# megapose6d/megapose6d

Measured on AMD Instinct MI355X. Metric: pose-hypotheses/sec (render+coarse+refine), 640×480, megapose-1.0-RGB, higher is better.
Workload: dtype f32 (results of fp32 arithmetic; the convolutions' multiplications run on the bf16 MFMA as EXACT piece products of the fp32 operands, fp32 accumulate)

## Files before the change

### megapose6d_amd/csrc/bf16x9_split.h

```cpp
#pragma once
#include <hip/hip_runtime.h>

#include <cstring>

namespace mp {

static inline void bf16x9_split3(float v, unsigned short out[3]) {
  unsigned vb, rb, qb;
  memcpy(&vb, &v, 4);
  const unsigned h = vb & 0xFFFF0000u;
  float hf; memcpy(&hf, &h, 4);
  const float r = v - hf;
  memcpy(&rb, &r, 4);
  const unsigned m = rb & 0xFFFF0000u;
  float mf; memcpy(&mf, &m, 4);
  const float q = r - mf;
  memcpy(&qb, &q, 4);
  out[0] = (unsigned short)(h >> 16); out[1] = (unsigned short)(m >> 16); out[2] = (unsigned short)(qb >> 16);
}

typedef unsigned bf16x9_u32x4 __attribute__((ext_vector_type(4)));

__device__ __forceinline__ void bf16x9_split8(const float4& lo, const float4& hi, bf16x9_u32x4 (&pc)[3]) {
  const float v[8] = {lo.x, lo.y, lo.z, lo.w, hi.x, hi.y, hi.z, hi.w};
  unsigned vb[8], rb[8], qb[8];
#pragma unroll
  for (int e = 0; e < 8; ++e) {
    vb[e] = __float_as_uint(v[e]);
    const float r = v[e] - __uint_as_float(vb[e] & 0xFFFF0000u);
    rb[e] = __float_as_uint(r);
    qb[e] = __float_as_uint(r - __uint_as_float(rb[e] & 0xFFFF0000u));
  }
#pragma unroll
  for (int j = 0; j < 4; ++j) {
    pc[0][j] = __builtin_amdgcn_perm(vb[2 * j + 1], vb[2 * j], 0x07060302u);
    pc[1][j] = __builtin_amdgcn_perm(rb[2 * j + 1], rb[2 * j], 0x07060302u);
    pc[2][j] = __builtin_amdgcn_perm(qb[2 * j + 1], qb[2 * j], 0x07060302u);
  }
}

}
```

### megapose6d_amd/csrc/conv_bf16x9.hip

```cpp
#include <cstdlib>

#include "bf16x9_split.h"
#include "conv_common.h"

namespace mp {

typedef __bf16 bf16x8 __attribute__((ext_vector_type(8)));
typedef bf16x9_u32x4 db_u32x4;

constexpr int DB_BM = 128, DB_BN = 128;
constexpr int DB_SLICE_BYTES = (DB_BN / 32) * 3 * 1024;
__device__ constexpr int DB_PA[9] = {2, 1, 2, 0, 1, 2, 0, 1, 0}, DB_PB[9] = {2, 2, 1, 2, 1, 0, 1, 0, 0};

__global__ __launch_bounds__(256) __attribute__((amdgpu_waves_per_eu(2, 2))) void conv_nhwc_bf16x9(ConvParams p) {
  __shared__ __attribute__((aligned(16))) float As[2 * DB_BM * LDS_LD];
  __shared__ int row_off[DB_BM];
  const int tid = threadIdx.x, lane = tid & 63;
  const int wave = __builtin_amdgcn_readfirstlane(tid >> 6);
  const int wm = wave >> 1, wn = wave & 1;
  const int lb = xcd_remap(blockIdx.x, gridDim.x);
  const int nblk = lb % p.n_nblocks, mblk = lb / p.n_nblocks;
  const int m0 = mblk * DB_BM, n0 = nblk * DB_BN;

  if (tid < DB_BM) {
    const int m = m0 + tid;
    int off = -1;
    if (m < p.M) {
      const int wo = m % p.Wo, t = m / p.Wo, ho = t % p.Ho, n = t / p.Ho;
      off = (((n * p.Hop) + ho + p.out_border) * p.Wop + wo + p.out_border) * p.Cout;
    }
    row_off[tid] = off;
  }
  const int a_c4 = tid & 7, a_r0 = tid >> 3;
  size_t pix[5];
#pragma unroll
  for (int i = 0; i < 5; ++i) {
    int m = i < 4 ? m0 + a_r0 + 32 * i : m0;
    m = m < p.M ? m : p.M - 1;
    const int wo = m % p.Wo, t = m / p.Wo, ho = t % p.Ho, n = t / p.Ho;
    pix[i] = ((size_t)n * p.Hp + (size_t)(ho * p.stride + p.in_off)) * p.Wp + (size_t)(wo * p.stride + p.in_off);
  }
  const __amdgpu_buffer_rsrc_t a_rsrc = __builtin_amdgcn_make_buffer_rsrc((void*)(p.x + pix[4] * p.C), 0, -1, 0x00020000);
  int a_voff[4];
#pragma unroll
  for (int i = 0; i < 4; ++i) a_voff[i] = (int)(((pix[i] - pix[4]) * p.C + a_c4 * 4) * 4);
  const __amdgpu_buffer_rsrc_t b_rsrc = __builtin_amdgcn_make_buffer_rsrc(
      (void*)(reinterpret_cast<const char*>(p.w) + (size_t)nblk * (2 * p.n_chunks) * DB_SLICE_BYTES), 0, -1, 0x00020000);
  const int b_voff = (2 * wn) * 3 * 1024 + lane * 16;

  f32x16 acc[2][2];
#pragma unroll
  for (int i = 0; i < 2; ++i)
#pragma unroll
    for (int j = 0; j < 2; ++j)
#pragma unroll
      for (int r = 0; r < 16; ++r) acc[i][j][r] = 0.f;

  float4 a0, a1, a2, a3;
  db_u32x4 bA[2][3], bB[2][3];
#define DB_BUF4(V, S) ([&] { const db_u32x4 v_ = __builtin_amdgcn_raw_buffer_load_b128(a_rsrc, V, S, 0);                  \
    return make_float4(__uint_as_float(v_.x), __uint_as_float(v_.y), __uint_as_float(v_.z), __uint_as_float(v_.w)); }())
#define DB_LOAD_A(SU)                       \
  a0 = DB_BUF4(a_voff[0], (SU) * 4);        \
  a1 = DB_BUF4(a_voff[1], (SU) * 4);        \
  a2 = DB_BUF4(a_voff[2], (SU) * 4);        \
  a3 = DB_BUF4(a_voff[3], (SU) * 4);
#define DB_LOAD_B(DST, SLICE)                                                                                       \
  _Pragma("unroll") for (int jl = 0; jl < 2; ++jl)                                                                  \
    _Pragma("unroll") for (int pc = 0; pc < 3; ++pc)                                                                \
      DST[jl][pc] = __builtin_amdgcn_raw_buffer_load_b128(b_rsrc, b_voff, (SLICE) * DB_SLICE_BYTES + (jl * 3 + pc) * 1024, 0);
#define DB_STORE_A(BUF)                                                            \
  {                                                                                \
    float* as_w = As + (BUF) * DB_BM * LDS_LD + a_r0 * LDS_LD + a_c4 * 4;          \
    *reinterpret_cast<float4*>(as_w) = a0;                                         \
    *reinterpret_cast<float4*>(as_w + 32 * LDS_LD) = a1;                           \
    *reinterpret_cast<float4*>(as_w + 64 * LDS_LD) = a2;                           \
    *reinterpret_cast<float4*>(as_w + 96 * LDS_LD) = a3;                           \
  }
#define DB_MFMA_SLICE(PA_, BB_)                                                                                     \
  _Pragma("unroll") for (int pr = 0; pr < 9; ++pr)                                                                  \
    _Pragma("unroll") for (int i = 0; i < 2; ++i)                                                                   \
      _Pragma("unroll") for (int j = 0; j < 2; ++j)                                                                 \
        acc[i][j] = __builtin_amdgcn_mfma_f32_32x32x16_bf16(__builtin_bit_cast(bf16x8, PA_[i][DB_PA[pr]]),          \
                                                            __builtin_bit_cast(bf16x8, BB_[j][DB_PB[pr]]), acc[i][j], 0, 0, 0);

  int a_su = 0, ju = 0;
  const int row_wrap = p.Wp * p.C - p.run;
  const int n_ch = p.n_chunks, last_slice = 2 * p.n_chunks - 1;
  DB_LOAD_A(0)
  DB_LOAD_B(bA, 0)
  DB_STORE_A(0)
  __syncthreads();

  const float* fr = As + (wm * 64 + (lane & 31)) * LDS_LD + (lane >> 5) * 8;
  for (int c = 0; c < n_ch; ++c) {
    const int buf = c & 1;
    if (c + 1 < n_ch) {
      a_su += BK;
      ju += BK;
      if (ju == p.run) { ju = 0; a_su += row_wrap; }
    }
    DB_LOAD_A(a_su)
    DB_LOAD_B(bB, 2 * c + 1)
    __builtin_amdgcn_sched_barrier(0);
    const float* fb = fr + buf * DB_BM * LDS_LD;
    float4 raw[2][2][2];
#pragma unroll
    for (int i = 0; i < 2; ++i) {
      raw[0][i][0] = *reinterpret_cast<const float4*>(fb + i * 32 * LDS_LD);
      raw[0][i][1] = *reinterpret_cast<const float4*>(fb + i * 32 * LDS_LD + 4);
    }
    db_u32x4 pa0[2][3], pa1[2][3];
    bf16x9_split8(raw[0][0][0], raw[0][0][1], pa0[0]);
    bf16x9_split8(raw[0][1][0], raw[0][1][1], pa0[1]);
    __builtin_amdgcn_sched_barrier(0);
#pragma unroll
    for (int i = 0; i < 2; ++i) {
      raw[1][i][0] = *reinterpret_cast<const float4*>(fb + i * 32 * LDS_LD + 16);
      raw[1][i][1] = *reinterpret_cast<const float4*>(fb + i * 32 * LDS_LD + 16 + 4);
    }
    DB_MFMA_SLICE(pa0, bA)
    bf16x9_split8(raw[1][0][0], raw[1][0][1], pa1[0]);
    bf16x9_split8(raw[1][1][0], raw[1][1][1], pa1[1]);
    __builtin_amdgcn_sched_group_barrier(0x100, 4, 0);
    __builtin_amdgcn_sched_group_barrier(0x008, 2, 0);
#pragma unroll
    for (int g = 0; g < 22; ++g) {
      __builtin_amdgcn_sched_group_barrier(0x002, 4, 0);
      __builtin_amdgcn_sched_group_barrier(0x008, 1, 0);
    }
    __builtin_amdgcn_sched_group_barrier(0x008, 12, 0);
    __builtin_amdgcn_sched_barrier(0);
    DB_LOAD_B(bA, (2 * c + 2 <= last_slice ? 2 * c + 2 : last_slice))
    DB_MFMA_SLICE(pa1, bB)
    DB_STORE_A(buf ^ 1)
    __syncthreads();
  }
#undef DB_BUF4
#undef DB_LOAD_A
#undef DB_LOAD_B
#undef DB_STORE_A
#undef DB_MFMA_SLICE

  const int erow0 = wm * 64 + (lane >> 5) * 4, en0 = n0 + wn * 64 + (lane & 31);
  const int emode = (p.residual ? 1 : 0) | (p.relu ? 2 : 0) | (p.y_act ? 4 : 0);
  switch (emode) {
    case 0: conv_epilogue<2, 2, false, false, false>(p, acc, row_off, erow0, en0); break;
    case 1: conv_epilogue<2, 2, true, false, false>(p, acc, row_off, erow0, en0); break;
    case 2: conv_epilogue<2, 2, false, true, false>(p, acc, row_off, erow0, en0); break;
    case 3: conv_epilogue<2, 2, true, true, false>(p, acc, row_off, erow0, en0); break;
    case 4: conv_epilogue<2, 2, false, false, true>(p, acc, row_off, erow0, en0); break;
    case 5: conv_epilogue<2, 2, true, false, true>(p, acc, row_off, erow0, en0); break;
    case 6: conv_epilogue<2, 2, false, true, true>(p, acc, row_off, erow0, en0); break;
    default: conv_epilogue<2, 2, true, true, true>(p, acc, row_off, erow0, en0); break;
  }
}

static int packed_slices(int Cin_p, int KH, int KW) { return 2 * ceil_div((long)KH * KW * Cin_p, BK); }

}

using namespace mp;

extern "C" size_t mp_conv_bf16x9_packed_bytes(int Cin_p, int Cout, int KH, int KW) {
  return (size_t)ceil_div(Cout, DB_BN) * packed_slices(Cin_p, KH, KW) * DB_SLICE_BYTES;
}

extern "C" int mp_conv_bf16x9_pack_weights(const float* w, int Cout, int Cin, int KH, int KW, int Cin_p, const float* scale, void* packed) {
  MP_REQUIRE(w && packed && Cout >= 1 && Cin >= 1 && KH >= 1 && KW >= 1 && Cin_p >= Cin && Cin_p % 16 == 0,
             "mp_conv_bf16x9_pack_weights: bad arguments (Cin_p %% 16 == 0, Cin_p >= Cin)");
  const int run = KW * Cin_p, k_total = KH * run, n_sl = packed_slices(Cin_p, KH, KW);
  unsigned short* out = (unsigned short*)packed;
  memset(out, 0, mp_conv_bf16x9_packed_bytes(Cin_p, Cout, KH, KW));
  for (int n = 0; n < Cout; ++n) {
    const float s = scale ? scale[n] : 1.f;
    const int nb = n / DB_BN, j = (n % DB_BN) / 32, nl = n % 32;
    for (int k = 0; k < k_total; ++k) {
      const int kh = k / run, jj = k % run, kw = jj / Cin_p, c = jj % Cin_p;
      if (c >= Cin) continue;
      unsigned short pc[3];
      bf16x9_split3(w[(((size_t)n * Cin + c) * KH + kh) * KW + kw] * s, pc);
      const int t = k / 16, lane = ((k % 16) / 8) * 32 + nl, e = k % 8;
      for (int piece = 0; piece < 3; ++piece)
        out[(((((size_t)nb * n_sl + t) * 4 + j) * 3 + piece) * 64 + lane) * 8 + e] = pc[piece];
    }
  }
  return MP_OK;
}

extern "C" int mp_conv2d_bf16x9_nhwc(const mp_conv_desc* desc, const void* d_w_pieces, mp_stream stream) {
  MP_REQUIRE(desc && d_w_pieces, "mp_conv2d_bf16x9_nhwc: null pointer");
  MP_REQUIRE(!desc->x_f16, "mp_conv2d_bf16x9_nhwc: fp32 input only");
  mp_conv_desc d = *desc;
  d.d_w = (const float*)d_w_pieces;
  ConvParams p;
  const int rc = conv_make_params(&d, &p);
  if (rc) return rc;
  MP_REQUIRE(d.C % 16 == 0 && p.run % BK == 0, "mp_conv2d_bf16x9_nhwc: needs C %% 16 == 0 and KW * C %% 32 == 0 (C = %d, KW = %d)", d.C, d.KW);
  p.n_mblocks = ceil_div(p.M, DB_BM);
  p.n_nblocks = ceil_div(p.Cout, DB_BN);
  const long n_tiles = (long)p.n_mblocks * p.n_nblocks;
  MP_REQUIRE(n_tiles < (1L << 31), "mp_conv2d_bf16x9_nhwc: grid too large");
  hipStream_t s = (hipStream_t)stream;
  const double M = p.M, alg_k = (double)d.KH * d.KW * (d.c_real > 0 ? d.c_real : d.C);
  ProfScope prof("conv_nhwc_bf16x9<128,128,64,64>", 2.0 * M * p.Cout * alg_k,
                 4.0 * (M * p.stride * p.stride * p.C + M * p.Cout) + 6.0 * (double)p.n_chunks * BK * p.n_nblocks * DB_BN, s,
                 9.0 * 2.0 * M * p.Cout * (double)p.n_chunks * BK, 2500.0);
  hipLaunchKernelGGL(conv_nhwc_bf16x9, dim3((unsigned)n_tiles), dim3(256), 0, s, p);
  MP_CHECK_HIP(hipGetLastError());
  return MP_OK;
}
```

Baseline: 2267.

## Split A tile into bf16 pieces once at LDS store with swizzled layout

Moves the fp32-to-three-bf16 splitting of the activation tile from the MFMA consumer side to the global-to-LDS staging step. Each element is now split once per block, not once per wave that reads it, and the pieces are stored as three swizzled bf16 planes that waves read directly as MFMA operands. The main loop is software-pipelined, with a peeled final iteration, early B prefetch, and new sched_group_barrier interleaving of MFMAs with LDS reads and writes. LDS footprint per buffer changes from fp32 rows to three bf16 planes, and the hand-tuned schedule counts may not match what the compiler emits.

```diff
diff --git a/megapose6d_amd/csrc/bf16x9_split.h b/megapose6d_amd/csrc/bf16x9_split.h
--- a/megapose6d_amd/csrc/bf16x9_split.h
+++ b/megapose6d_amd/csrc/bf16x9_split.h
@@ -20,19 +20,20 @@
 }
 
 typedef unsigned bf16x9_u32x4 __attribute__((ext_vector_type(4)));
+typedef unsigned bf16x9_u32x2 __attribute__((ext_vector_type(2)));
 
-__device__ __forceinline__ void bf16x9_split8(const float4& lo, const float4& hi, bf16x9_u32x4 (&pc)[3]) {
-  const float v[8] = {lo.x, lo.y, lo.z, lo.w, hi.x, hi.y, hi.z, hi.w};
-  unsigned vb[8], rb[8], qb[8];
+__device__ __forceinline__ void bf16x9_split4(const float4& v4, bf16x9_u32x2 (&pc)[3]) {
+  const float v[4] = {v4.x, v4.y, v4.z, v4.w};
+  unsigned vb[4], rb[4], qb[4];
 #pragma unroll
-  for (int e = 0; e < 8; ++e) {
+  for (int e = 0; e < 4; ++e) {
     vb[e] = __float_as_uint(v[e]);
     const float r = v[e] - __uint_as_float(vb[e] & 0xFFFF0000u);
     rb[e] = __float_as_uint(r);
     qb[e] = __float_as_uint(r - __uint_as_float(rb[e] & 0xFFFF0000u));
   }
 #pragma unroll
-  for (int j = 0; j < 4; ++j) {
+  for (int j = 0; j < 2; ++j) {
     pc[0][j] = __builtin_amdgcn_perm(vb[2 * j + 1], vb[2 * j], 0x07060302u);
     pc[1][j] = __builtin_amdgcn_perm(rb[2 * j + 1], rb[2 * j], 0x07060302u);
     pc[2][j] = __builtin_amdgcn_perm(qb[2 * j + 1], qb[2 * j], 0x07060302u);
diff --git a/megapose6d_amd/csrc/conv_bf16x9.hip b/megapose6d_amd/csrc/conv_bf16x9.hip
--- a/megapose6d_amd/csrc/conv_bf16x9.hip
+++ b/megapose6d_amd/csrc/conv_bf16x9.hip
@@ -7,13 +7,15 @@
 
 typedef __bf16 bf16x8 __attribute__((ext_vector_type(8)));
 typedef bf16x9_u32x4 db_u32x4;
+typedef bf16x9_u32x2 db_u32x2;
 
 constexpr int DB_BM = 128, DB_BN = 128;
 constexpr int DB_SLICE_BYTES = (DB_BN / 32) * 3 * 1024;
+constexpr int DB_ROW_BYTES = BK * 2, DB_PLANE_BYTES = DB_BM * DB_ROW_BYTES, DB_BUF_BYTES = 3 * DB_PLANE_BYTES;
 __device__ constexpr int DB_PA[9] = {2, 1, 2, 0, 1, 2, 0, 1, 0}, DB_PB[9] = {2, 2, 1, 2, 1, 0, 1, 0, 0};
 
 __global__ __launch_bounds__(256) __attribute__((amdgpu_waves_per_eu(2, 2))) void conv_nhwc_bf16x9(ConvParams p) {
-  __shared__ __attribute__((aligned(16))) float As[2 * DB_BM * LDS_LD];
+  __shared__ __attribute__((aligned(16))) unsigned char As[2 * DB_BUF_BYTES];
   __shared__ int row_off[DB_BM];
   const int tid = threadIdx.x, lane = tid & 63;
   const int wave = __builtin_amdgcn_readfirstlane(tid >> 6);
@@ -21,40 +23,6 @@
   const int lb = xcd_remap(blockIdx.x, gridDim.x);
   const int nblk = lb % p.n_nblocks, mblk = lb / p.n_nblocks;
   const int m0 = mblk * DB_BM, n0 = nblk * DB_BN;
-
-  if (tid < DB_BM) {
-    const int m = m0 + tid;
-    int off = -1;
-    if (m < p.M) {
-      const int wo = m % p.Wo, t = m / p.Wo, ho = t % p.Ho, n = t / p.Ho;
-      off = (((n * p.Hop) + ho + p.out_border) * p.Wop + wo + p.out_border) * p.Cout;
-    }
-    row_off[tid] = off;
-  }
-  const int a_c4 = tid & 7, a_r0 = tid >> 3;
-  size_t pix[5];
-#pragma unroll
-  for (int i = 0; i < 5; ++i) {
-    int m = i < 4 ? m0 + a_r0 + 32 * i : m0;
-    m = m < p.M ? m : p.M - 1;
-    const int wo = m % p.Wo, t = m / p.Wo, ho = t % p.Ho, n = t / p.Ho;
-    pix[i] = ((size_t)n * p.Hp + (size_t)(ho * p.stride + p.in_off)) * p.Wp + (size_t)(wo * p.stride + p.in_off);
-  }
-  const __amdgpu_buffer_rsrc_t a_rsrc = __builtin_amdgcn_make_buffer_rsrc((void*)(p.x + pix[4] * p.C), 0, -1, 0x00020000);
-  int a_voff[4];
-#pragma unroll
-  for (int i = 0; i < 4; ++i) a_voff[i] = (int)(((pix[i] - pix[4]) * p.C + a_c4 * 4) * 4);
-  const __amdgpu_buffer_rsrc_t b_rsrc = __builtin_amdgcn_make_buffer_rsrc(
-      (void*)(reinterpret_cast<const char*>(p.w) + (size_t)nblk * (2 * p.n_chunks) * DB_SLICE_BYTES), 0, -1, 0x00020000);
-  const int b_voff = (2 * wn) * 3 * 1024 + lane * 16;
-
-  f32x16 acc[2][2];
-#pragma unroll
-  for (int i = 0; i < 2; ++i)
-#pragma unroll
-    for (int j = 0; j < 2; ++j)
-#pragma unroll
-      for (int r = 0; r < 16; ++r) acc[i][j][r] = 0.f;
 
   float4 a0, a1, a2, a3;
   db_u32x4 bA[2][3], bB[2][3];
@@ -69,78 +37,142 @@
   _Pragma("unroll") for (int jl = 0; jl < 2; ++jl)                                                                  \
     _Pragma("unroll") for (int pc = 0; pc < 3; ++pc)                                                                \
       DST[jl][pc] = __builtin_amdgcn_raw_buffer_load_b128(b_rsrc, b_voff, (SLICE) * DB_SLICE_BYTES + (jl * 3 + pc) * 1024, 0);
-#define DB_STORE_A(BUF)                                                            \
-  {                                                                                \
-    float* as_w = As + (BUF) * DB_BM * LDS_LD + a_r0 * LDS_LD + a_c4 * 4;          \
-    *reinterpret_cast<float4*>(as_w) = a0;                                         \
-    *reinterpret_cast<float4*>(as_w + 32 * LDS_LD) = a1;                           \
-    *reinterpret_cast<float4*>(as_w + 64 * LDS_LD) = a2;                           \
-    *reinterpret_cast<float4*>(as_w + 96 * LDS_LD) = a3;                           \
-  }
-#define DB_MFMA_SLICE(PA_, BB_)                                                                                     \
-  _Pragma("unroll") for (int pr = 0; pr < 9; ++pr)                                                                  \
+#define DB_SPLIT_STORE_A(V_, I_, BUF)                                                                               \
+  {                                                                                                                 \
+    db_u32x2 sp_[3];                                                                                                \
+    bf16x9_split4(V_, sp_);                                                                                         \
+    _Pragma("unroll") for (int pc = 0; pc < 3; ++pc)                                                                \
+      *reinterpret_cast<db_u32x2*>(As + (BUF) * DB_BUF_BYTES + pc * DB_PLANE_BYTES + (I_) * 32 * DB_ROW_BYTES + a_wr) = sp_[pc];   \
+  }
+#define DB_STAGE_A(BUF)            \
+  DB_SPLIT_STORE_A(a0, 0, BUF)     \
+  DB_SPLIT_STORE_A(a1, 1, BUF)     \
+  DB_SPLIT_STORE_A(a2, 2, BUF)     \
+  DB_SPLIT_STORE_A(a3, 3, BUF)
+#define DB_READ_A(PA_, BUF, RD_)                                                                                    \
+  _Pragma("unroll") for (int i = 0; i < 2; ++i)                                                                     \
+    _Pragma("unroll") for (int pc = 0; pc < 3; ++pc)                                                                \
+      PA_[i][pc] = *reinterpret_cast<const db_u32x4*>(As + (BUF) * DB_BUF_BYTES + pc * DB_PLANE_BYTES + i * 32 * DB_ROW_BYTES + RD_);
+#define DB_MFMA_PAIRS(PA_, BB_, P0_, P1_)                                                                           \
+  _Pragma("unroll") for (int pr = P0_; pr < P1_; ++pr)                                                              \
     _Pragma("unroll") for (int i = 0; i < 2; ++i)                                                                   \
       _Pragma("unroll") for (int j = 0; j < 2; ++j)                                                                 \
         acc[i][j] = __builtin_amdgcn_mfma_f32_32x32x16_bf16(__builtin_bit_cast(bf16x8, PA_[i][DB_PA[pr]]),          \
                                                             __builtin_bit_cast(bf16x8, BB_[j][DB_PB[pr]]), acc[i][j], 0, 0, 0);
 
+  const __amdgpu_buffer_rsrc_t b_rsrc = __builtin_amdgcn_make_buffer_rsrc(
+      (void*)(reinterpret_cast<const char*>(p.w) + (size_t)nblk * (2 * p.n_chunks) * DB_SLICE_BYTES), 0, -1, 0x00020000);
+  const int b_voff = (2 * wn) * 3 * 1024 + lane * 16;
+  DB_LOAD_B(bA, 0)
+  const int a_c4 = tid & 7, a_r0 = tid >> 3;
+  size_t pix[5];
+#pragma unroll
+  for (int i = 0; i < 5; ++i) {
+    int m = i < 4 ? m0 + a_r0 + 32 * i : m0;
+    m = m < p.M ? m : p.M - 1;
+    const int wo = m % p.Wo, t = m / p.Wo, ho = t % p.Ho, n = t / p.Ho;
+    pix[i] = ((size_t)n * p.Hp + (size_t)(ho * p.stride + p.in_off)) * p.Wp + (size_t)(wo * p.stride + p.in_off);
+  }
+  const __amdgpu_buffer_rsrc_t a_rsrc = __builtin_amdgcn_make_buffer_rsrc((void*)(p.x + pix[4] * p.C), 0, -1, 0x00020000);
+  int a_voff[4];
+#pragma unroll
+  for (int i = 0; i < 4; ++i) a_voff[i] = (int)(((pix[i] - pix[4]) * p.C + a_c4 * 4) * 4);
+  DB_LOAD_A(0)
+  __builtin_amdgcn_sched_barrier(0);
+
+  if (tid < DB_BM) {
+    const int m = m0 + tid;
+    int off = -1;
+    if (m < p.M) {
+      const int wo = m % p.Wo, t = m / p.Wo, ho = t % p.Ho, n = t / p.Ho;
+      off = (((n * p.Hop) + ho + p.out_border) * p.Wop + wo + p.out_border) * p.Cout;
+    }
+    row_off[tid] = off;
+  }
+  const int a_wr = a_r0 * DB_ROW_BYTES + ((((a_c4 >> 1) ^ (a_r0 >> 2)) & 3) << 4) + ((a_c4 & 1) << 3);
+  const int a_rd0 = (wm * 64 + (lane & 31)) * DB_ROW_BYTES + ((((lane >> 5) ^ (lane >> 2)) & 3) << 4);
+  const int a_rd1 = a_rd0 ^ 32;
+
+  f32x16 acc[2][2];
+#pragma unroll
+  for (int i = 0; i < 2; ++i)
+#pragma unroll
+    for (int j = 0; j < 2; ++j)
+#pragma unroll
+      for (int r = 0; r < 16; ++r) acc[i][j][r] = 0.f;
+
   int a_su = 0, ju = 0;
   const int row_wrap = p.Wp * p.C - p.run;
-  const int n_ch = p.n_chunks, last_slice = 2 * p.n_chunks - 1;
-  DB_LOAD_A(0)
-  DB_LOAD_B(bA, 0)
-  DB_STORE_A(0)
+  const int n_ch = p.n_chunks;
+  db_u32x4 pa0[2][3], pa1[2][3];
+  DB_STAGE_A(0)
   __syncthreads();
-
-  const float* fr = As + (wm * 64 + (lane & 31)) * LDS_LD + (lane >> 5) * 8;
-  for (int c = 0; c < n_ch; ++c) {
+  DB_READ_A(pa0, 0, a_rd0)
+
+  for (int c = 0; c + 1 < n_ch; ++c) {
     const int buf = c & 1;
-    if (c + 1 < n_ch) {
-      a_su += BK;
-      ju += BK;
-      if (ju == p.run) { ju = 0; a_su += row_wrap; }
-    }
+    a_su += BK;
+    ju += BK;
+    if (ju == p.run) { ju = 0; a_su += row_wrap; }
     DB_LOAD_A(a_su)
     DB_LOAD_B(bB, 2 * c + 1)
     __builtin_amdgcn_sched_barrier(0);
-    const float* fb = fr + buf * DB_BM * LDS_LD;
-    float4 raw[2][2][2];
-#pragma unroll
-    for (int i = 0; i < 2; ++i) {
-      raw[0][i][0] = *reinterpret_cast<const float4*>(fb + i * 32 * LDS_LD);
-      raw[0][i][1] = *reinterpret_cast<const float4*>(fb + i * 32 * LDS_LD + 4);
-    }
-    db_u32x4 pa0[2][3], pa1[2][3];
-    bf16x9_split8(raw[0][0][0], raw[0][0][1], pa0[0]);
-    bf16x9_split8(raw[0][1][0], raw[0][1][1], pa0[1]);
-    __builtin_amdgcn_sched_barrier(0);
-#pragma unroll
-    for (int i = 0; i < 2; ++i) {
-      raw[1][i][0] = *reinterpret_cast<const float4*>(fb + i * 32 * LDS_LD + 16);
-      raw[1][i][1] = *reinterpret_cast<const float4*>(fb + i * 32 * LDS_LD + 16 + 4);
-    }
-    DB_MFMA_SLICE(pa0, bA)
-    bf16x9_split8(raw[1][0][0], raw[1][0][1], pa1[0]);
-    bf16x9_split8(raw[1][1][0], raw[1][1][1], pa1[1]);
-    __builtin_amdgcn_sched_group_barrier(0x100, 4, 0);
-    __builtin_amdgcn_sched_group_barrier(0x008, 2, 0);
-#pragma unroll
-    for (int g = 0; g < 22; ++g) {
-      __builtin_amdgcn_sched_group_barrier(0x002, 4, 0);
-      __builtin_amdgcn_sched_group_barrier(0x008, 1, 0);
-    }
-    __builtin_amdgcn_sched_group_barrier(0x008, 12, 0);
-    __builtin_amdgcn_sched_barrier(0);
-    DB_LOAD_B(bA, (2 * c + 2 <= last_slice ? 2 * c + 2 : last_slice))
-    DB_MFMA_SLICE(pa1, bB)
-    DB_STORE_A(buf ^ 1)
+    DB_READ_A(pa1, buf, a_rd1)
+    DB_MFMA_PAIRS(pa0, bA, 0, 9)
+    __builtin_amdgcn_sched_group_barrier(0x008, 1, 0);
+#pragma unroll
+    for (int g = 0; g < 6; ++g) {
+      __builtin_amdgcn_sched_group_barrier(0x100, 1, 0);
+      __builtin_amdgcn_sched_group_barrier(0x008, 1, 0);
+    }
+    __builtin_amdgcn_sched_group_barrier(0x008, 29, 0);
+    __builtin_amdgcn_sched_barrier(0);
+    DB_LOAD_B(bA, 2 * c + 2)
+    __builtin_amdgcn_sched_barrier(0);
+    DB_MFMA_PAIRS(pa1, bB, 0, 7)
+    DB_STAGE_A(buf ^ 1)
+#pragma unroll
+    for (int g = 0; g < 4; ++g) {
+#pragma unroll
+      for (int h = 0; h < 5; ++h) {
+        __builtin_amdgcn_sched_group_barrier(0x008, 1, 0);
+        __builtin_amdgcn_sched_group_barrier(0x002, 4, 0);
+      }
+      __builtin_amdgcn_sched_group_barrier(0x008, 1, 0);
+      __builtin_amdgcn_sched_group_barrier(0x002, 2, 0);
+      __builtin_amdgcn_sched_group_barrier(0x200, 1, 0);
+      __builtin_amdgcn_sched_group_barrier(0x008, 1, 0);
+      __builtin_amdgcn_sched_group_barrier(0x200, 2, 0);
+    }
+    __builtin_amdgcn_sched_barrier(0);
     __syncthreads();
+    DB_READ_A(pa0, buf ^ 1, a_rd0)
+    DB_MFMA_PAIRS(pa1, bB, 7, 9)
+    __builtin_amdgcn_sched_barrier(0);
+  }
+  {
+    const int c = n_ch - 1;
+    DB_LOAD_B(bB, 2 * c + 1)
+    __builtin_amdgcn_sched_barrier(0);
+    DB_READ_A(pa1, c & 1, a_rd1)
+    DB_MFMA_PAIRS(pa0, bA, 0, 9)
+    __builtin_amdgcn_sched_group_barrier(0x008, 1, 0);
+#pragma unroll
+    for (int g = 0; g < 6; ++g) {
+      __builtin_amdgcn_sched_group_barrier(0x100, 1, 0);
+      __builtin_amdgcn_sched_group_barrier(0x008, 1, 0);
+    }
+    __builtin_amdgcn_sched_group_barrier(0x008, 29, 0);
+    __builtin_amdgcn_sched_barrier(0);
+    DB_MFMA_PAIRS(pa1, bB, 0, 9)
   }
 #undef DB_BUF4
 #undef DB_LOAD_A
 #undef DB_LOAD_B
-#undef DB_STORE_A
-#undef DB_MFMA_SLICE
+#undef DB_SPLIT_STORE_A
+#undef DB_STAGE_A
+#undef DB_READ_A
+#undef DB_MFMA_PAIRS
 
   const int erow0 = wm * 64 + (lane >> 5) * 4, en0 = n0 + wn * 64 + (lane & 31);
   const int emode = (p.residual ? 1 : 0) | (p.relu ? 2 : 0) | (p.y_act ? 4 : 0);
```

Measured after the change: 2256. Within noise of the previous version (-0.5%).
